# Xtra-Computing/FedTree

Hardware: AMD Instinct MI355X
Metric: Paillier-2048 encrypts/s device-resident; ciphertext adds/s; 1/2/4/8 GPU (higher is better)
Workload: dtype u32

## Files before the change

### fedtree_amd/build.py

```python
#!/usr/bin/env python3
import hashlib
import os
import subprocess
import sys

HERE = os.path.dirname(os.path.abspath(__file__))
CSRC = os.path.join(HERE, "csrc")
GEN = os.path.join(CSRC, "gen")
LLVM = "/opt/rocm/lib/llvm/bin"
ARCH = "gfx950"
VARIANTS = ((37, 28, 12, False), (74, 28, 12, False), (152, 27, 4, True), (80, 27, 4, True))
DEFAULT_OUT = os.path.join(HERE, "libfthe.so")
OUT = os.path.abspath(os.environ.get("FTHE_BUILD_OUT") or DEFAULT_OUT)


def run(cmd):
    r = subprocess.run(cmd, capture_output=True, text=True)
    if r.returncode != 0:
        sys.stderr.write(" ".join(cmd) + "\n" + r.stdout + r.stderr)
        raise SystemExit(r.returncode)
    return r


def build_kernels():
    os.makedirs(GEN, exist_ok=True)
    sys.path.insert(0, CSRC)
    if OUT == DEFAULT_OUT:
        for k in sorted(k for k in os.environ if k.startswith("FTHE_GEN_")):
            os.environ.pop(k)
            sys.stderr.write(f"build.py: ignoring {k} (A/B generator switch) for the in-tree library\n")
    import gen_montprog
    import gen_padic
    import gen_nadic
    import gen_padic_mfma
    import gen_addb
    import gen_nadicb
    for lay_name, new_lay in (("addb_layout.h", gen_addb.layout_header()), ("nadicb_layout.h", gen_nadicb.layout_header())):
        lay = os.path.join(GEN, lay_name)
        if not os.path.exists(lay) or open(lay).read() != new_lay:
            with open(lay, "w") as f:
                f.write(new_lay)
    blobs = []
    kernels = [(S, f"fthe_montprog_s{S}", f"montprog_s{S}",
                (lambda S=S, B=B, U=U, quad=quad, n=f"fthe_montprog_s{S}":
                 (gen_montprog.gen_quad if quad else gen_montprog.gen)(S, B, U, n)))
               for S, B, U, quad in VARIANTS]
    for K in (37, 19):
        kernels.append((1000 + K, f"fthe_padic_k{K}", f"padic_k{K}",
                        lambda K=K: gen_padic.gen_padic(K, 28, f"fthe_padic_k{K}")))
    kernels.append((1137, "fthe_padic_m37", "padic_m37", lambda: gen_padic_mfma.gen_padic_mfma("fthe_padic_m37")))
    kernels.append((1237, "fthe_padic_m37t", "padic_m37t",
                    lambda: gen_padic_mfma.gen_padic_mfma("fthe_padic_m37t", top_est=True)))
    kernels.append((2076, "fthe_nadic_q76", "nadic_q76", lambda: gen_nadic.gen_nadic(76, 27, "fthe_nadic_q76")))
    kernels.append((2176, "fthe_nadic_m76", "nadic_m76",
                    lambda: gen_nadic.gen_nadic(76, 27, "fthe_nadic_m76", mont=True)))
    kernels.append((2276, "fthe_nadic_b76", "nadic_b76", lambda: gen_nadicb.gen_nadicb("fthe_nadic_b76")))
    kernels.append((3152, "fthe_addb_q152", "addb_q152", lambda: gen_addb.gen_addb("fthe_addb_q152")))
    for S, name, stem, make in kernels:
        asm = os.path.join(GEN, f"{stem}.s")
        src = make()
        old = open(asm).read() if os.path.exists(asm) else None
        if old != src:
            with open(asm, "w") as f:
                f.write(src)
        obj = os.path.join(GEN, f"{stem}.o")
        hsaco = os.path.join(GEN, f"{stem}.hsaco")
        run([f"{LLVM}/clang", "-x", "assembler", "-target", "amdgcn-amd-amdhsa", f"-mcpu={ARCH}",
             "-c", asm, "-o", obj])
        run([f"{LLVM}/ld.lld", "-shared", obj, "-o", hsaco])
        blobs.append((S, open(hsaco, "rb").read()))
    hdr = ["// generated by fedtree_amd/build.py -- gfx950 code objects of the montprog kernels",
           "#pragma once", "#include <cstddef>", ""]
    for S, b in blobs:
        hdr.append(f"alignas(64) static const unsigned char fthe_blob_s{S}[{len(b)}] = {{")
        for i in range(0, len(b), 24):
            hdr.append("  " + ",".join(str(x) for x in b[i:i + 24]) + ",")
        hdr.append("};")
    hdr.append("static inline const unsigned char *fthe_montprog_blob(int S) {")
    for S, _ in blobs:
        hdr.append(f"  if (S == {S}) return fthe_blob_s{S};")
    hdr.append("  return nullptr;")
    hdr.append("}")
    path = os.path.join(GEN, "montprog_blobs.h")
    new = "\n".join(hdr) + "\n"
    if not os.path.exists(path) or open(path).read() != new:
        with open(path, "w") as f:
            f.write(new)


def build_lib():
    srcs = [os.path.join(CSRC, "fthe.hip"), os.path.join(CSRC, "fthe_glue.hip"), os.path.join(CSRC, "fthe_hist.hip"),
            os.path.join(CSRC, "fthe_dec.hip"), os.path.join(CSRC, "fthe_wire.cpp")]
    deps = srcs + [os.path.join(CSRC, f) for f in ("bn_host.hpp", "fthe_glue.h", "padic_tiles.hpp", "addb_image.hpp",
                                                    "nadicb_image.hpp")] + \
        [os.path.join(GEN, "montprog_blobs.h"), os.path.join(GEN, "addb_layout.h"), os.path.join(GEN, "nadicb_layout.h"),
         os.path.join(HERE, "..", "include", "fthe.h")]
    cmd = ["/opt/rocm/bin/hipcc", f"--offload-arch={ARCH}", "-O3", "-fPIC", "-shared", "-std=c++17",
           "-idirafter", "/opt/conda/include", "-Wno-unused-result",
           *(["-DFTHE_STAMP_HOOK"] if OUT != DEFAULT_OUT else []),
           *srcs, "-l:libgmp.so.10", "-o", OUT + ".tmp"]
    h = hashlib.sha256(" ".join(cmd[:-2]).encode())
    for d in deps:
        with open(d, "rb") as f:
            h.update(os.path.basename(d).encode() + b"\0" + f.read())
    digest = h.hexdigest()
# ... 18 lines not shown
```

### fedtree_amd/csrc/fthe.hip

```cpp
#include <hip/hip_runtime.h>
#include <cstdio>
#include <cstdlib>
#include <cstring>
#include <algorithm>
#include <atomic>
#include <cmath>
#include <chrono>
#include <condition_variable>
#include <functional>
#include <map>
#include <memory>
#include <string>
#include <mutex>
#include <new>
#include <random>
#include <thread>
#include <unordered_map>
#include <vector>
#include <fcntl.h>
#include <unistd.h>

#include "../../include/fthe.h"
#include "bn_host.hpp"
#include "padic_tiles.hpp"
#include "addb_image.hpp"
#include "nadicb_image.hpp"
#include "fthe_glue.h"
#include "gen/montprog_blobs.h"

using namespace fthe;

#define HIPOK(x) do { if ((x) != hipSuccess) return FTHE_ERR_HIP; } while (0)

namespace {

constexpr int MAX_VARIANTS = 11;
constexpr int kPadicS = 1037, kPadicK = 37, kPadicSmallK = 19, kNadicS = 2076, kPadicMfmaS = 1137,
              kNadicMontS = 2176, kNadicBarS = 2276, kPadicMfmaTS = 1237;
constexpr int kPadicTopBits = 1027, kPadicPtShift = 1000, kPadicPtWord = 100;
const Shape kVariants[MAX_VARIANTS] = {{37, 28, 1}, {74, 28, 1}, {152, 27, 4}, {80, 27, 4},
                                       {1000 + kPadicK, 28, 1}, {1000 + kPadicSmallK, 28, 1}, {kNadicS, 27, 4},
                                       {kPadicMfmaS, 28, 1}, {kNadicMontS, 27, 4}, {kNadicBarS, 27, 4},
                                       {kPadicMfmaTS, 28, 1}};
constexpr Shape kLatShape{80, 27, 4};
constexpr int kAddbBlob = 3152;

int variant_index(int S) {
    for (int i = 0; i < MAX_VARIANTS; i++) if (kVariants[i].S == S) return i;
    return -1;
}

void urandom_bytes(void *dst, size_t n) {
    uint8_t *p = (uint8_t *)dst;
    size_t got = 0;
    int fd = open("/dev/urandom", O_RDONLY);
    if (fd >= 0) {
        while (got < n) {
            ssize_t r = read(fd, p + got, n - got);
            if (r <= 0) break;
            got += (size_t)r;
        }
        close(fd);
    }
    if (got < n) {
        std::random_device rd;
        for (; got < n; got++) p[got] = (uint8_t)rd();
    }
}

uint64_t splitmix64(uint64_t &s) {
    uint64_t z = (s += 0x9E3779B97F4A7C15ull);
    z = (z ^ (z >> 30)) * 0xBF58476D1CE4E5B9ull;
    z = (z ^ (z >> 27)) * 0x94D049BB133111EBull;
    return z ^ (z >> 31);
}

RngKey make_rng_key(uint64_t seed, uint64_t tweak) {
    RngKey rk{};
    if (!seed) {
        urandom_bytes(rk.k, sizeof rk.k);
        urandom_bytes(&rk.nonce, sizeof rk.nonce);
        return rk;
    }
    uint64_t s = seed;
    for (int i = 0; i < 8; i += 2) { uint64_t v = splitmix64(s); rk.k[i] = (uint32_t)v; rk.k[i + 1] = (uint32_t)(v >> 32); }
    rk.nonce = splitmix64(s) ^ tweak;
    return rk;
}

void seed_gmp_state(gmp_randstate_t st, uint64_t seed, uint64_t tweak) {
    Mpz sd;
    if (!seed) {
        uint32_t w[8];
        urandom_bytes(w, sizeof w);
        mpz_import(sd, 8, -1, 4, 0, 0, w);
    } else {
// ... 330 lines not shown
static bool lds_prefetch(const Shape &sh) {
    static const bool off = getenv("FTHE_NO_LDSDMA") != nullptr;
    return sh.lanes == 1 && !off;
}

extern "C" int fthe_version(void) { return 100; }

extern "C" const char *fthe_strerror(int s) {
    switch (s) {
        case FTHE_OK: return "ok";
        case FTHE_ERR_ARG: return "invalid argument";
        case FTHE_ERR_HIP: return "HIP runtime error (no gfx950 device or launch failure)";
        case FTHE_ERR_NOPRIV: return "private key required";
        case FTHE_ERR_UNSUPPORTED: return "modulus size not supported by the built kernels";
        case FTHE_ERR_KEY: return "invalid key material";
        case FTHE_ERR_NOMEM: return "device allocation failed";
        default: return "unknown status";
    }
}

extern "C" int fthe_kernel_limbs(int bits) { return kernel_limbs_for_bits(bits); }

extern "C" int fthe_device_count(void) {
    int n = 0;
    return hipGetDeviceCount(&n) == hipSuccess && n > 0 ? n : 0;
}

extern "C" int fthe_ctx_create(int device, fthe_ctx **out) {
    if (!out) return FTHE_ERR_ARG;
    *out = nullptr;
    int ndev = 0;
    if (hipGetDeviceCount(&ndev) != hipSuccess || ndev <= 0 || device < 0 || device >= ndev) return FTHE_ERR_HIP;
    HIPOK(hipSetDevice(device));
    std::unique_ptr<fthe_ctx> c(new fthe_ctx);
    c->device = device;
    HIPOK(hipStreamCreateWithFlags(&c->stream, hipStreamNonBlocking));
    HIPOK(hipStreamCreateWithFlags(&c->copy, hipStreamNonBlocking));
    HIPOK(hipStreamCreateWithFlags(&c->side, hipStreamNonBlocking));
    HIPOK(hipEventCreateWithFlags(&c->ev_fork, hipEventDisableTiming));
    HIPOK(hipEventCreateWithFlags(&c->ev_join, hipEventDisableTiming));
    for (int i = 0; i < 2; i++) {
        HIPOK(hipEventCreateWithFlags(&c->ev_done[i], hipEventDisableTiming));
        HIPOK(hipEventCreateWithFlags(&c->ev_copied[i], hipEventDisableTiming));
        HIPOK(hipEventCreateWithFlags(&c->ev_in[i], hipEventDisableTiming));
    }
    for (int i = 0; i < MAX_VARIANTS; i++) {
        const unsigned char *blob = fthe_montprog_blob(kVariants[i].S);
        if (!blob) return FTHE_ERR_HIP;
        HIPOK(hipModuleLoadData(&c->mod[i], blob));
        char name[64];
        if (kVariants[i].S > 2200) snprintf(name, sizeof name, "fthe_nadic_b%d", kVariants[i].S - 2200);
        else if (kVariants[i].S > 2100) snprintf(name, sizeof name, "fthe_nadic_m%d", kVariants[i].S - 2100);
        else if (kVariants[i].S > 2000) snprintf(name, sizeof name, "fthe_nadic_q%d", kVariants[i].S - 2000);
        else if (kVariants[i].S > 1200) snprintf(name, sizeof name, "fthe_padic_m%dt", kVariants[i].S - 1200);
        else if (kVariants[i].S > 1100) snprintf(name, sizeof name, "fthe_padic_m%d", kVariants[i].S - 1100);
        else if (kVariants[i].S > 1000) snprintf(name, sizeof name, "fthe_padic_k%d", kVariants[i].S - 1000);
        else snprintf(name, sizeof name, "fthe_montprog_s%d", kVariants[i].S);
        HIPOK(hipModuleGetFunction(&c->fn[i], c->mod[i], name));
        HIPOK(hipFuncGetAttribute(&c->static_lds[i], HIP_FUNC_ATTRIBUTE_SHARED_SIZE_BYTES, c->fn[i]));
    }
    if (const unsigned char *blob = fthe_montprog_blob(kAddbBlob)) {
        HIPOK(hipModuleLoadData(&c->mod_addb, blob));
        HIPOK(hipModuleGetFunction(&c->fn_addb, c->mod_addb, "fthe_addb_q152"));
    }
    HIPOK(hipEventCreate(&c->ev0));
    HIPOK(hipEventCreate(&c->ev1));
    HIPOK(hipDeviceGetAttribute(&c->n_cu, hipDeviceAttributeMultiprocessorCount, device));
    *out = c.release();
    return FTHE_OK;
}

extern "C" int fthe_host_alloc(size_t bytes, void **out) {
    if (!out) return FTHE_ERR_ARG;
    *out = nullptr;
    if (bytes == 0) return FTHE_OK;
    if (hipHostMalloc(out, bytes, hipHostMallocDefault) != hipSuccess) { *out = nullptr; return FTHE_ERR_HIP; }
    return FTHE_OK;
}

extern "C" void fthe_host_free(void *p) {
    if (p) (void)hipHostFree(p);
}

extern "C" void fthe_ctx_destroy(fthe_ctx *c) {
    if (!c) return;
    (void)hipSetDevice(c->device);
    if (c->stream) (void)hipStreamSynchronize(c->stream);
    if (c->copy) (void)hipStreamSynchronize(c->copy);
    if (c->side) (void)hipStreamSynchronize(c->side);
    for (int i = 0; i < MAX_VARIANTS; i++) if (c->mod[i]) (void)hipModuleUnload(c->mod[i]);
    if (c->mod_addb) (void)hipModuleUnload(c->mod_addb);
    if (c->d_jobctr) (void)hipFree(c->d_jobctr);
    if (c->cub_tmp) (void)hipFree(c->cub_tmp);
    for (auto &e : c->prof_ev) { (void)hipEventDestroy(e.first); (void)hipEventDestroy(e.second); }
    if (c->ev0) (void)hipEventDestroy(c->ev0);
    if (c->ev1) (void)hipEventDestroy(c->ev1);
    if (c->stream) (void)hipStreamDestroy(c->stream);
    if (c->copy) (void)hipStreamDestroy(c->copy);
    if (c->side) (void)hipStreamDestroy(c->side);
    if (c->ev_fork) (void)hipEventDestroy(c->ev_fork);
    if (c->ev_join) (void)hipEventDestroy(c->ev_join);
    for (int i = 0; i < 2; i++) {
        if (c->ev_done[i]) (void)hipEventDestroy(c->ev_done[i]);
        if (c->ev_copied[i]) (void)hipEventDestroy(c->ev_copied[i]);
        if (c->ev_in[i]) (void)hipEventDestroy(c->ev_in[i]);
    }
// ... 24 lines not shown
}
extern "C" double fthe_last_montmuls(fthe_ctx *c) { return c ? c->last_mm : 0.0; }

extern "C" int fthe_prof_variant(fthe_ctx *c, int S, double *expo_ms, double *expo_launches) {
    if (!c) return FTHE_ERR_ARG;
    int vi = variant_index(S);
    if (vi < 0) return FTHE_ERR_ARG;
    if (expo_ms) *expo_ms = c->var_ms[vi];
    if (expo_launches) *expo_launches = c->var_n[vi];
    return FTHE_OK;
}

extern "C" int fthe_prof_enable(fthe_ctx *c, int on) {
    if (!c) return FTHE_ERR_ARG;
    c->prof = on != 0;
    c->prof_used = 0; c->prof_lane_mm = 0; c->prof_launch_lanes = 0; c->prof_alg_macs = 0;
    c->prof_exec_macs = 0;
    return FTHE_OK;
}

extern "C" int fthe_prof_busy(fthe_ctx *c, double *busy_ms, double *expo_busy_ms) {
    if (!c) return FTHE_ERR_ARG;
    if (busy_ms) *busy_ms = c->prof_busy_ms;
    if (expo_busy_ms) *expo_busy_ms = c->prof_expo_busy_ms;
    return FTHE_OK;
}

extern "C" int fthe_prof_exec_macs(fthe_ctx *c, double *exec_macs) {
    if (!c || !exec_macs) return FTHE_ERR_ARG;
    HIPOK(hipSetDevice(c->device));
    HIPOK(hipStreamSynchronize(c->stream));
    *exec_macs = c->prof_exec_macs;
    return FTHE_OK;
}

extern "C" int fthe_prof_read(fthe_ctx *c, double *kernel_ms, double *launches, double *lane_montmuls, double *lanes,
                              double *expo_ms, double *expo_launches, double *alg_macs) {
    if (!c) return FTHE_ERR_ARG;
    HIPOK(hipSetDevice(c->device));
    HIPOK(hipStreamSynchronize(c->stream));
    HIPOK(hipStreamSynchronize(c->side));
    double tot = 0, etot = 0, en = 0;
    for (int v = 0; v < MAX_VARIANTS; v++) c->var_ms[v] = c->var_n[v] = 0;
    std::vector<std::pair<double, double>> iv, eiv;
    for (size_t i = 0; i < c->prof_used; i++) {
        float ms = 0, t0 = 0;
        HIPOK(hipEventElapsedTime(&ms, c->prof_ev[i].first, c->prof_ev[i].second));
        HIPOK(hipEventElapsedTime(&t0, c->prof_ev[0].first, c->prof_ev[i].first));
        tot += ms;
        iv.emplace_back(t0, (double)t0 + ms);
        if (c->prof_mm[i] >= 64) {
            etot += ms; en += 1;
            c->var_ms[c->prof_vi[i]] += ms; c->var_n[c->prof_vi[i]] += 1;
            if (kVariants[c->prof_vi[i]].S == kPadicMfmaTS) {
                const int vm = variant_index(kPadicMfmaS);
                c->var_ms[vm] += ms; c->var_n[vm] += 1;
            }
            eiv.emplace_back(t0, (double)t0 + ms);
        }
    }
    auto union_ms = [](std::vector<std::pair<double, double>> &v) {
        std::sort(v.begin(), v.end());
        double u = 0, a = 0, b = -1e300;
        for (auto &x : v) {
            if (x.first > b) { if (b > a) u += b - a; a = x.first; b = x.second; }
            else b = std::max(b, x.second);
        }
        if (!v.empty() && b > a) u += b - a;
        return u;
    };
    c->prof_busy_ms = union_ms(iv);
    c->prof_expo_busy_ms = union_ms(eiv);
    if (kernel_ms) *kernel_ms = tot;
    if (expo_ms) *expo_ms = etot;
    if (expo_launches) *expo_launches = en;
    if (launches) *launches = (double)c->prof_used;
    if (lane_montmuls) *lane_montmuls = c->prof_lane_mm;
    if (lanes) *lanes = c->prof_launch_lanes;
    if (alg_macs) *alg_macs = c->prof_alg_macs;
    c->prof_used = 0; c->prof_lane_mm = 0; c->prof_launch_lanes = 0; c->prof_alg_macs = 0; c->prof_exec_macs = 0;
    return FTHE_OK;
}

static int upload_mod(DevMod &d, const mpz_t N, Shape sh) {
    d.m.init(N, sh);
    if (hipMalloc(&d.d_ctx, d.m.ctx.size() * 4) != hipSuccess) return FTHE_ERR_NOMEM;
    HIPOK(hipMemcpy(d.d_ctx, d.m.ctx.data(), d.m.ctx.size() * 4, hipMemcpyHostToDevice));
    return FTHE_OK;
}

static int padic_digits(const mpz_t P, Shape sh) {
    if (getenv("FTHE_NO_PADIC") || sh.B != 28 || sh.lanes != 1) return 0;
    const size_t b = mpz_sizeinbase(P, 2);
    if (sh.S == 2 * kPadicK && b >= 1009 && b <= 1030) return kPadicK;
    if (sh.S == 37 && b >= 505 && b <= 516) return kPadicSmallK;
    return 0;
}
static int upload_padic(DevMod &d, const mpz_t P, int K) {
    Mpz P2; mpz_mul(P2, P, P);
    d.m.init(P2, Shape{2 * K, 28, 1});
    const int pad = ((20 + K + 3) & ~3) - 20 - K;
    std::vector<uint8_t> tiles;
    if (K == kPadicK && !getenv("FTHE_NO_PADIC_MFMA")) tiles = padic_tiles::build(P);
    std::vector<uint32_t> w(tiles.empty() ? (size_t)2 * K + 1 + pad : 128 + tiles.size() / 4, 0u), l = to_limbs(P, K, 28);
    if (!tiles.empty()) std::memcpy(w.data() + 128, tiles.data(), tiles.size());
    for (int j = 0; j < K; j++) w[j] = (uint32_t)(-(int32_t)l[j]);
    Mpz mu; mpz_set_ui(mu, 1); mpz_mul_2exp(mu, mu, 56 * K); mpz_fdiv_q(mu, mu, P);
    std::vector<uint32_t> ml = to_limbs(mu, K + 1, 28);
    std::copy(ml.begin(), ml.end(), w.begin() + K + pad);
    if (!tiles.empty()) {
        static_assert(kPadicPtWord >= 2 * kPadicK + 1 + 3 && kPadicPtWord < 128, "Pt between mu and the tile image");
        Mpz pt; mpz_fdiv_q_2exp(pt, P, kPadicPtShift);
        w[kPadicPtWord] = (uint32_t)mpz_get_ui(pt);
    }
    if (hipMalloc(&d.d_ctx, w.size() * 4) != hipSuccess) return FTHE_ERR_NOMEM;
    HIPOK(hipMemcpy(d.d_ctx, w.data(), w.size() * 4, hipMemcpyHostToDevice));
    d.kernel_S = 1000 + K;
    const bool top_est = !tiles.empty() && mpz_sizeinbase(P, 2) <= (size_t)kPadicTopBits && !getenv("FTHE_NO_M37T");
    d.kernel_S_mfma = tiles.empty() ? 0 : top_est ? kPadicMfmaTS : kPadicMfmaS;
    return FTHE_OK;
}
static double padic_alg(const Prog &p, const mpz_t P) {
    const double s = (double)((mpz_sizeinbase(P, 2) + 31) / 32);
    const double bar = (s + 1) * (s + 2) / 2 + s * (s + 1) / 2;
    const double sq = s * s + s * (s + 1) / 2 + 2 * bar, mul = 3 * s * s + 2 * bar;
    return p.squarings * sq + (p.montmuls - p.squarings) * mul + bar + s * s;
}
static double padic_exec(const Prog &p, int Kd) {
    const double K = Kd;
    const double bar = K * (K + 1) + 3 * K + 1;
    const double sq = K * K + K * (K + 1) / 2 + 2 * bar, mul = 3 * K * K + 2 * bar;
    return p.squarings * sq + (p.montmuls - p.squarings) * mul + bar + K * K + K;
}

constexpr Shape kNadicDigit{76, 27, 4};
static bool nadic_ok(const fthe_key *k) {
    const size_t b = mpz_sizeinbase(k->n, 2);
    return !getenv("FTHE_NO_NADIC") && k->sn2.S == 152 && k->sn2.B == 27 && k->sn2.lanes == 4 &&
           b >= 2042 && b <= 2050;
}
static bool nadic_mont_ok(const fthe_key *k) {
    return !getenv("FTHE_NO_NADIC") && !getenv("FTHE_NADIC_CLASSICAL") && k->sn2.S == 152 && k->sn2.B == 27 &&
           k->sn2.lanes == 4 && mpz_sizeinbase(k->n, 2) <= 2048;
}
static bool nadicb_ok(const fthe_key *k) {
    return !getenv("FTHE_NO_NADIC") && !getenv("FTHE_NADIC_MONT") && !getenv("FTHE_NADIC_CLASSICAL") &&
           k->sn2.S == 152 && k->sn2.B == 27 && k->sn2.lanes == 4 && nadicb::n_ok(k->n);
}
static int upload_nadic(DevMod &d, const mpz_t n, const mpz_t n2, Shape slots, bool classical = true) {
    d.m.init(n2, slots);
    MontMod dm;
    dm.init(n, kNadicDigit);
    if (classical && !dm.classical_ok()) return FTHE_ERR_UNSUPPORTED;
    if (hipMalloc(&d.d_ctx, dm.ctx.size() * 4) != hipSuccess) return FTHE_ERR_NOMEM;
    HIPOK(hipMemcpy(d.d_ctx, dm.ctx.data(), dm.ctx.size() * 4, hipMemcpyHostToDevice));
    d.kernel_S = kNadicS;
    return FTHE_OK;
}
static double nadic_alg(const Prog &p, const mpz_t n) {
    const double s = (double)((mpz_sizeinbase(n, 2) + 31) / 32);
    return p.squarings * 4 * s * s + (p.montmuls - p.squarings) * 5 * s * s;
}
static double nadic_exec(const Prog &p) {
    return p.squarings * 76.0 * 76 + (p.montmuls - p.squarings) * 76.0 * 95;
}

static int key_finish(fthe_key *k) {
    if (k->priv) {
        Mpz p2; mpz_mul(p2, k->p, k->p);
        Mpz q2; mpz_mul(q2, k->q, k->q);
        size_t b = std::max(p2.bits(), q2.bits());
        k->spq = kernel_shape_for_bits((int)b);
// ... 3294 lines not shown
```

### fedtree_amd/csrc/gen_padic_mfma.py

```python
#!/usr/bin/env python3
import os
import sys

sys.path.insert(0, os.path.dirname(os.path.abspath(__file__)))
from gen_montprog import _descriptor

AB = os.environ.get("FTHE_GEN_M37_AB", "")
TILE_OFF = 512
TILE_BYTES = 20 * 1024
SPILL_BYTES = 10 * 1024
SPILL = "spill" in AB
PP = "pingpong" in AB
MARGIN = next((int(t[6:]) for t in AB.split(',') if t.startswith('margin') and t[6:].isdigit()), 30)
assert MARGIN >= 24
PREXOR = "noprexor" not in AB
CMERGE = "nocmerge" not in AB
LDSX = "ldsx" in AB
LDSXA = LDSX and "ldsxa" in AB
LDSX_BYTES = 5 * 1024
KARA = "nokara" not in AB
assert not (KARA and LDSX)
assert not (LDSX and (PP or SPILL))
LDS_BYTES = TILE_BYTES + (4 * SPILL_BYTES if SPILL else 0) + (4 * LDSX_BYTES if LDSX else 0)
S1_LO = 112 if "s1lo112" in AB else 128
S1_TOP = 272
Q3DW = "noq3dw" not in AB and not LDSX
QBIT = 28 * 38
TILE_D1 = (-3, -2, -1, 0, 1)
TILE_D2 = (0, 1, 2, 3)


def tile_index(prod, m, k):
    if prod == 1:
        return TILE_D1.index(m - k) if k <= 3 else 5 + m
    return 10 + m if k == 0 else 15 + TILE_D2.index(m - k)


TOPEST_MAX_BITS = 1027
PT_OFF = 400
PT_SHIFT = 1000
TOPEST_C = 128 << 8


def gen_padic_mfma(name: str, top_est: bool = False) -> str:
    K, B = 37, 28
    MASK = (1 << B) - 1
    V_TID, V_GOFF = 0, 1
    VA = (2, 6, 10)
    NCOL = next((int(t[3:]) for t in AB.split(',') if t in ('col3', 'col4')), 2)
    assert NCOL == 2 or not KARA, "col3 / col4 predate the Karatsuba cross term (wrong results, r06s): add nokara"
    ACC0 = 10 if NCOL == 2 else 2
    CARRY = ACC0 + 4 * NCOL
    XA = 20
    G0, G1 = XA, XA + 16
    XB = 60
    TT = 100
    VV = 174
    V_LDS = 248
    V_SPILL = 249
    PATV = (249, 250)
    assert not (SPILL and PREXOR)
    NVGPR = 250 if SPILL else 251 if PREXOR else 249
    V_XW, V_XR = NVGPR, NVGPR + 1
    if LDSX:
        NVGPR += 2

    def pat(t):
        return f"v{PATV[t % 2]}"
    PATVAL = (0x00808080, 0x08080808)
    X0 = [f"v{XA + i}" for i in range(K)]
    X1 = [f"v{XB + i}" for i in range(K)]
    T = [f"v{TT + i}" for i in range(2 * K)]
    V = [f"v{VV + i}" for i in range(2 * K)]
    D = [f"v{XB + i}" for i in range(40)]
    SPOW, SNEG, SNP = 20, 28, 36
    NSGPR = SNP + K
    SLO, SHI = 74, 76
    if LDSX:
        NSGPR = SHI + 2
    if KARA:
        NSGPR = 79
    SPT = NSGPR
    if top_est:
        NSGPR += 1
    POW = lambda sh: f"s{SPOW + sh // 4}"
    NEG = lambda sh: f"s{SNEG + sh // 4}"
    NP = lambda j: f"s{SNP + j}"

    def pair(n):
        return f"v[{n}:{n + 1}]"

    def acc(s, ch):
        n = ACC0 + 2 * (NCOL * s + ch)
        return f"v[{n}:{n + 1}]"

    def acclo(s, ch):
        return f"v{ACC0 + 2 * (NCOL * s + ch)}"

    carry = pair(CARRY)
# ... 77 lines not shown
            used = [False] * len(seqs)
            for ci in range(gi + NCOL, min(gi + 2 * NCOL, len(cols))):
                pending += list(cols[ci].get('pre', ()))
            n = 0
            for t in range(max(len(q[1]) for q in seqs)):
                for k, (ac, terms, add) in enumerate(seqs):
                    if t < len(terms):
                        a_, b_ = terms[t]
                        e(f'  {mad} {ac}, vcc, {a_}, {b_}, {ac if used[k] else (add or "0")}')
                        used[k] = True
                        n += 1
                        if n % 2 == 0:
                            tick()
            flush(len(pending))
            tail = []
            for m, ci in enumerate(members):
                tail += tail_of(ci, cols[ci], acc(s, m), acclo(s, m), used[m])
            pending = tail
        flush(len(pending))
        for ins in bgq:
            e(ins)

    def product_cols(a, b, n_out, outs, a2=None, b2=None):
        cols = []
        for c in range(n_out):
            terms = []
            for i in range(len(a)):
                j = c - i
                if 0 <= j < len(b):
                    terms.append((a[i], b[j]))
                    if a2 is not None:
                        terms.append((a2[i], b2[j]))
            cols.append({'terms': terms, 'out': outs[c], 'last': c == n_out - 1})
            if PREXOR and c >= K:
                cols[-1]['px'] = pat(c - (K - 1))
        return cols

    def move(dst, src):
        n = len(src)
        for i in range(0, n - 1, 2):
            if int(dst[i][1:]) % 2 == 0 and int(src[i][1:]) % 2 == 0:
                e(f'  v_pk_mov_b32 {pair(int(dst[i][1:]))}, {pair(int(src[i][1:]))}, {pair(int(src[i][1:]))} op_sel:[0,1]')
            else:
                e(f'  v_mov_b32_e32 {dst[i]}, {src[i]}')
                e(f'  v_mov_b32_e32 {dst[i + 1]}, {src[i + 1]}')
        if n % 2:
            e(f'  v_mov_b32_e32 {dst[n - 1]}, {src[n - 1]}')

    CACC2 = (pair(XA + 32), pair(XA + 34))
    CCARRY = pair(XA + 38)
    SMASK = "s35"
    S2MASK, S3MASK, S4MASK = "s76", "s77", "s78"

    def orpack(limbs, shift_bits, ndw, xor_masks, lead_one=False, norm0=False, pre=()):
        n = len(limbs)
        pre = set(pre)

        def carried(w):
            m = 0
            for b in range(32):
                q = 32 * w - shift_bits + b
                if q < 0 or (lead_one and w == 0 and b < 8):
                    continue
                t, j = q // B, q % B
                if t in pre and t < n and (PATVAL[t % 2] >> j) & 1:
                    m |= 1 << b
            return m
        xor_masks = [xor_masks[w] ^ carried(w) for w in range(ndw)]
        for w in range(ndw):
            d = D[w]
            if lead_one and w == 0:
                e(f'  v_lshl_or_b32 {d}, {limbs[0]}, 8, 1')
            else:
                lo = (32 * w - shift_bits) // B
                off = 32 * w - shift_bits - B * lo
                hi_ok = lo + 1 < n
                if norm0 and lo == 0:
                    assert off == 0 and hi_ok
                    e(f'  v_lshlrev_b32_e32 {d}, 28, {limbs[1]}')
                    e(f'  v_bfi_b32 {d}, {SMASK}, {limbs[0]}, {d}')
                elif not hi_ok:
                    e(f'  v_lshrrev_b32_e32 {d}, {off}, {limbs[lo]}')
                elif off == 0:
                    e(f'  v_lshl_or_b32 {d}, {limbs[lo + 1]}, 28, {limbs[lo]}')
                else:
                    e(f'  v_lshrrev_b32_e32 {d}, {off}, {limbs[lo]}')
                    e(f'  v_lshl_or_b32 {d}, {limbs[lo + 1]}, {B - off}, {d}')
            if xor_masks[w]:
                e(f'  v_xor_b32_e32 {d}, {hex(xor_masks[w])}, {d}')

    D2 = [f"v{VV + 38 + i}" for i in range(36)] + [f"v{16 + i}" for i in range(4)]
    OPND = [D]

    def swap_operands(Dl=D, nk=5):
        if LDSX:
            assert nk == 5
            lo, hi = f"s[{SLO}:{SLO + 1}]", f"s[{SHI}:{SHI + 1}]"
            e(f'  s_mov_b64 exec, {lo}')
            for k in range(5):
                e(f'  ds_write_b128 v{V_XW}, v[{XB + 8 * k + 4}:{XB + 8 * k + 7}] offset:{1024 * k}')
            e(f'  s_mov_b64 exec, {hi}')
            for k in range(5):
                e(f'  ds_write_b128 v{V_XW}, v[{XB + 8 * k}:{XB + 8 * k + 3}] offset:{1024 * k}')
            for k in range(5):
                e(f'  ds_read_b128 v[{XB + 8 * k}:{XB + 8 * k + 3}], v{V_XR} offset:{1024 * k}')
            e(f'  s_mov_b64 exec, {lo}')
            for k in range(5):
                e(f'  ds_read_b128 v[{XB + 8 * k + 4}:{XB + 8 * k + 7}], v{V_XR} offset:{1024 * k}')
            e('  s_mov_b64 exec, -1')
            return
        e('  s_nop 1')
        for k in range(nk):
            for j in range(4):
                e(f'  v_permlane32_swap_b32_e32 {Dl[8 * k + j]}, {Dl[8 * k + 4 + j]}')
        e('  s_nop 4')

    def rd(prod, m, k, n):
        b_ = VA[n % 3]
        e(f'  ds_read_b128 v[{b_}:{b_ + 3}], v{V_LDS} offset:{1024 * tile_index(prod, m, k)}')

    def prefetch(prod, m, ks):
        for n in range(min(2, len(ks))):
            rd(prod, m, ks[n], n)

    GB0, GB1 = TT + 38, TT + 54
    GV0, GV1 = VV + 38, VV + 54

    def issue_tile(prod, m, ks, G0x, G1x, prefetched=True):
        L = len(ks)
        if not prefetched:
            prefetch(prod, m, ks)
        for n, k in enumerate(ks):
            if n + 2 < L:
                rd(prod, m, ks[n + 2], n + 2)
            e(f'  s_waitcnt lgkmcnt({min(L, n + 3) - n - 1})')
            buf = VA[n % 3]
            for g, G in ((0, G0x), (1, G1x)):
                src_c = "0" if n == 0 else f"v[{G}:{G + 15}]"
                bo = 8 * k + 4 * g
                b0 = int(OPND[0][bo][1:])
                assert b0 % 2 == 0 and [int(r[1:]) for r in OPND[0][bo:bo + 4]] == list(range(b0, b0 + 4))
                if "nomfma" not in AB:
                    e(f'  v_mfma_i32_32x32x32_i8 v[{G}:{G + 15}], v[{buf}:{buf + 3}], v[{b0}:{b0 + 3}], {src_c}')

    P1_TOP = [S1_TOP]

    def consumed(prod, m):
        if prod == 1:
            return {rho for rho in range(32) if S1_LO + 32 * m + rho < P1_TOP[0]}
        return {rho for rho in range(32) if 1 <= 32 * m + rho <= 130}

    def plan(C):
        paired, swaps = set(), []
        for rr in range(0, 16, 2):
            ra = 8 * (rr >> 2) + (rr & 3)
            rhos = (ra, ra + 4)
            if "noprepair" not in AB and all((r in C) == (r + 1 in C) for r in rhos) \
                    and any(r in C for r in rhos):
                paired.add(rr)
        for rr in range(16):
            ra = 8 * (rr >> 2) + (rr & 3)
            if (ra in C or ra + 4 in C) and not (rr % 2 and rr - 1 in paired):
                swaps.append(rr)
        return paired, swaps

    def compact(tile):
        return LDSXA and plan(consumed(*tile))[0] == set(range(0, 16, 2))

    def exchange(G0x, G1x, waited=False, tile=None):
        if "nonop" not in AB and not waited:
            e('  s_nop 7')
            e('  s_nop 7')
# ... 143 lines not shown
                tail += self.out(self.t, f'v{a[2:a.index(":")]}')
            elif 0 <= self.t < len(self.outs):
                if self.px:
                    tail.append(f'  v_bitop3_b32 {self.outs[self.t]}, v{a[2:a.index(":")]}, {SMASK}, '
                                f'{pat(self.t)} bitop3:0x6a')
                else:
                    tail.append(f'  v_and_b32_e32 {self.outs[self.t]}, {hex(MASK)}, v{a[2:a.index(":")]}')
            if not (self.nocarry_last and self.t == self.t_last):
                if CMERGE:
                    e(f'  v_ashrrev_i64 {CCARRY}, {self.radix}, {a}')
                else:
                    tail.append(f'  v_ashrrev_i64 {CCARRY}, {self.radix}, {a}')
            self.pending = tail
            self.t += 1
            self.fresh = True
            if self.t <= self.t_last:
                self.start()

        def column(self, s, reg):
            t = (8 * s - self.base) // self.radix
            while t > self.t:
                self.close()
            if not self.begun:
                self.begun = True
                self.start()
            sh = 8 * s - self.base - self.radix * t
            mul = NEG(sh) if self.neg else POW(sh)
            a = self.acc()
            self.emit(f'  v_mad_i64_i32 {a}, vcc, {reg}, {mul}, {self.addend0() if self.fresh else a}')
            self.fresh = False

        def finish(self):
            while self.t <= self.t_last:
                self.close()
            for ins in self.pending:
                e(ins)
            self.pending = []

    def fold_columns(ch, cols):
        i = 0
        while i < len(cols):
            s_, r_, pr_ = cols[i]
            if not pr_ and i + 1 < len(cols) and "nopair" not in AB:
                s2_, r2_, pr2_ = cols[i + 1]
                t1, t2 = (8 * s_ - ch.base) // ch.radix, (8 * s2_ - ch.base) // ch.radix
                if not pr2_ and s2_ == s_ + 1 and t1 == t2 and 8 * s_ - ch.base - ch.radix * t1 <= 16:
                    e(f'  v_lshl_add_u32 {r_}, {r2_}, 8, {r_}')
                    ch.column(s_, r_)
                    i += 2
                    continue
            ch.column(s_, r_)
            i += 1

    P1_TILES = [(1, m, [k for k in range(5) if m - k <= 1]) for m in range(5)]
    P2_TILES = [(2, m, [k for k in range(5) if m >= k]) for m in range(5)]
    assert P1_TILES[0][2][0] != 4 and P2_TILES[0][2][0] != 4

    V_FRAC = XA + 37
    assert V_FRAC not in range(G0, G0 + 32) and V_FRAC not in range(XA + 32, XA + 37) and \
        V_FRAC not in (XA + 38, XA + 39) and V_FRAC < XB and V_FRAC >= CARRY + 2 and V_FRAC not in VA

    def mfma_barrett(Tl, q3out, clamp, prefetched=False, dbuf=False, setb=None, pre_in=None, dw=None, t4=False):
        if pre_in is None:
            pre_in = PREXOR
        if not prefetched:
            prefetch(*P1_TILES[0])
        orpack(Tl[K - 1:2 * K], 0, 34, [0x80808080] * 34, norm0=True, pre=range(1, K + 1) if pre_in else ())
        e(f'  v_bfe_u32 {D[34]}, {Tl[K - 1]}, 28, 1')
        e(f'  v_lshl_or_b32 {D[34]}, {D[34]}, 12, 1')
        for w in range(35, 40):
            e(f'  v_mov_b32_e32 {D[w]}, 0')
        swap_operands()
        if dw is None:
            tap = {-1: lambda lo: [f'  v_lshlrev_b32_e32 v{V_FRAC}, 4, {lo}']} if t4 else None
            ch = Chunks(QBIT, (8 * S1_LO - QBIT) // B, 39, q3out, neg=False, px=PREXOR, tap=tap)
        else:
            assert not clamp
            base = QBIT - 8

            ndw = 32 if t4 else 33
            tap = {-1: lambda lo: [f'  v_mov_b32_e32 v{V_FRAC}, {lo}'],
                   0: lambda lo: [f'  v_alignbit_b32 v{V_FRAC}, {lo}, v{V_FRAC}, 8']} if t4 else None

            def out(w, lo):
                if w < 0:
                    return []
                if w == 0:
                    return [f'  v_and_b32_e32 {dw[0]}, 0xffffff00, {lo}', f'  v_xor_b32_e32 {dw[0]}, 0x80808001, {dw[0]}']
                if w == 32:
                    return [f'  v_and_b32_e32 {dw[32]}, {hex((1 << (B * K + 8 - 1024)) - 1)}, {lo}',
                            f'  v_xor_b32_e32 {dw[32]}, 0x80808080, {dw[32]}']
                return [f'  v_xor_b32_e32 {dw[w]}, 0x80808080, {lo}']
            ch = Chunks(base, (8 * S1_LO - base) // 32, ndw - 1, None, neg=False, nocarry_last=True, radix=32,
                        out=out, tap=tap)
            P1_TOP[0] = (base + ndw * 32) // 8

        def consume(m, creg):
            fold_columns(ch, tile_cols(1, m, lambda rho: S1_LO + 32 * m + rho, creg))
        run_tiles(P1_TILES, consume, P2_TILES[0], dbuf, setb=setb)
        ch.finish()
        P1_TOP[0] = S1_TOP
        if clamp:
            e(f'  v_not_b32_e32 v{XA + 36}, v{XA + 38}')
            for t, r in enumerate(q3out):
                if PREXOR:
                    e(f'  v_bitop3_b32 {r}, {r}, v{XA + 36}, {pat(t)} bitop3:0xe2')
                else:
                    e(f'  v_and_b32_e32 {r}, {r}, v{XA + 36}')
        return q3out

    def mfma_remainder(Tl, q3, rout, nxt_p1, dbuf=False, after_pack=None, dw=None, t4=False, clamped=False):
        Dl = D if dw is None else dw
        nk = 4 if t4 else 5
        if dw is None:
            orpack(q3, 8, 32 if t4 else 33, [0x80808000] + [0x80808080] * 32, lead_one=True,
                   pre=range(K) if PREXOR else ())
        if after_pack and not dbuf:
            after_pack()
        if not t4:
            e(f'  v_mov_b32_e32 {Dl[33]}, 0x80')
            for w in range(34, 40):
                e(f'  v_mov_b32_e32 {Dl[w]}, 0')
        swap_operands(Dl, nk)
        OPND[0] = Dl
# ... 343 lines not shown
        e('  s_waitcnt vmcnt(0)')
        e('.Lstamp_done:')
    e('  s_endpgm')

    e('.Lreduce:')
    PRIO = next((int(t[4:]) for t in AB.split(',') if t.startswith('prio') and t[4:].isdigit()),
                0 if "noprio" in AB else 3)
    if PRIO:
        e(f'  s_setprio {PRIO}')
    dbuf = "nodbuf" not in AB
    spill = dbuf and SPILL
    if spill:
        for j in range(9):
            e(f'  ds_write_b128 v{V_SPILL}, v[{VV + 38 + 4 * j}:{VV + 41 + 4 * j}] offset:{1024 * j}')
        e(f'  ds_write_b32 v{V_SPILL}, {V[K]} offset:{9 * 1024}')
    q3 = mfma_barrett(T, T[K:], clamp=True, dbuf=spill, setb=(GV0, GV1), t4=top_est)

    def add_u1():
        for i in range(K):
            if PREXOR:
                e(f'  v_xad_u32 {V[i]}, {q3[i]}, {pat(i)}, {V[i]}')
            else:
                e(f'  v_add_u32_e32 {V[i]}, {V[i]}, {q3[i]}')
        if spill:
            for j in range(9):
                e(f'  ds_read_b128 v[{VV + 38 + 4 * j}:{VV + 41 + 4 * j}], v{V_SPILL} offset:{1024 * j}')
            e(f'  ds_read_b32 {V[K]}, v{V_SPILL} offset:{9 * 1024}')
    mfma_remainder(T, q3, T[:K], nxt_p1=True, dbuf=dbuf, after_pack=add_u1, t4=top_est, clamped=True)
    if Q3DW:
        mfma_barrett(V, None, clamp=False, prefetched=True, dbuf=dbuf, dw=D2, t4=top_est)
        mfma_remainder(V, None, V[:K], nxt_p1=False, dbuf=dbuf, dw=D2, t4=top_est)
    else:
        q3b = mfma_barrett(V, V[K:], clamp=False, prefetched=True, dbuf=dbuf, t4=top_est)
        mfma_remainder(V, q3b, V[:K], nxt_p1=False, dbuf=dbuf, t4=top_est)
    move(X0, T[:K])
    move(X1, V[:K])
    if PRIO:
        e('  s_setprio 0')
    e('  s_setpc_b64 s[12:13]')

    e(f'.Lfunc_end_{name}:')
    e(f'  .size {name}, .Lfunc_end_{name}-{name}')
    e('')
    o.extend(_descriptor(name, LDS_BYTES, NVGPR, 98 if DYN else 90 if STAMP else NSGPR,
                         max_wg=512 if PP else 256).splitlines())
    return "\n".join(o) + "\n"


if __name__ == "__main__":
    import argparse
    ap = argparse.ArgumentParser()
    ap.add_argument('--name', default='fthe_padic_m37')
    ap.add_argument('--top-est', action='store_true', help='the four-tile body (fthe_padic_m37t)')
    ap.add_argument('-o', '--out', required=True)
    a = ap.parse_args()
    with open(a.out, 'w') as f:
        f.write(gen_padic_mfma(a.name, top_est=a.top_est))
```

### fedtree_amd/csrc/padic_tiles.hpp

```cpp
#pragma once
#include <gmp.h>
#include <cstdint>
#include <vector>

namespace padic_tiles {

constexpr int kTiles = 19, kImageBytes = 20 * 1024, kS1Lo = 128, kNq1 = 136, kConst1 = 136, kNq3 = 132;

inline bool balanced(const mpz_t x, int n, std::vector<int> &d) {
    mpz_t t;
    mpz_init_set(t, x);
    d.assign(n, 0);
    int c = 0;
    for (int k = 0; k < n; k++) {
        int v = (int)(mpz_get_ui(t) & 255u) + c;
        mpz_fdiv_q_2exp(t, t, 8);
        if (v >= 128) { d[k] = v - 256; c = 1; } else { d[k] = v; c = 0; }
    }
    bool ok = mpz_sgn(t) == 0 && c == 0;
    mpz_clear(t);
    return ok;
}

inline void offset_sum(mpz_t out, const mpz_t x, int n) {
    mpz_t g;
    mpz_init(g);
    mpz_ui_pow_ui(g, 256, (unsigned long)n);
    mpz_sub_ui(g, g, 1);
    mpz_divexact_ui(g, g, 255);
    mpz_mul(out, g, x);
    mpz_mul_ui(out, out, 128);
    mpz_clear(g);
}

inline std::vector<uint8_t> build(const mpz_t P, int s1lo = kS1Lo) {
    std::vector<uint8_t> img;
    if (mpz_sizeinbase(P, 2) < 1009 || mpz_sizeinbase(P, 2) > 1030) return img;
    if (s1lo != 112 && s1lo != 128) return img;
    mpz_t mu, c, b;
    mpz_inits(mu, c, b, nullptr);
    mpz_set_ui(mu, 1);
    mpz_mul_2exp(mu, mu, 56 * 37);
    mpz_fdiv_q(mu, mu, P);
    std::vector<int> mud, pd, g1, g2;
    bool ok = balanced(mu, 135, mud) && balanced(P, 130, pd);
    offset_sum(c, mu, kNq1);
    mpz_set_ui(b, 1);
    mpz_mul_2exp(b, b, 8 * s1lo + 22);
    mpz_sub(c, c, b);
    mpz_fdiv_q_2exp(c, c, 8 * s1lo);
    ok = ok && balanced(c, 160, g1);
    offset_sum(c, P, kNq3);
    mpz_fdiv_r_2exp(c, c, 1040);
    ok = ok && balanced(c, 131, g2);
    mpz_clears(mu, c, b, nullptr);
    if (!ok) return img;
    g2.resize(130);
    auto a1 = [&](int s, int i) -> int {
        if (i == kConst1) return (s >= s1lo && s < s1lo + 160) ? g1[s - s1lo] : 0;
        if (i == kConst1 + 1) {
            int j = s - 3;
            return (j >= 0 && j < (int)mud.size()) ? mud[j] : 0;
        }
        if (i > kConst1) return 0;
        int j = s - i;
        return (j >= 0 && j < (int)mud.size()) ? mud[j] : 0;
    };
    auto a2 = [&](int s, int i) -> int {
        if (i == 0) return (s >= 1 && s <= (int)g2.size()) ? g2[s - 1] : 0;
        int j = s - i;
        return (j >= 0 && j < (int)pd.size()) ? pd[j] : 0;
    };
    img.reserve(kImageBytes);
    auto tile = [&](int prod, int s_base, int m, int k) {
        for (int l = 0; l < 64; l++) {
            const int r = l & 31, h = l >> 5;
            for (int j = 0; j < 16; j++) {
                const int s = s_base + 32 * m + r, i = 32 * k + 16 * h + j;
                img.push_back((uint8_t)((prod == 1 ? a1(s, i) : a2(s, i)) & 255));
            }
        }
    };
    for (int d = -3; d <= 1; d++) tile(1, s1lo, d >= 0 ? d : 0, d >= 0 ? 0 : -d);
    for (int m = 0; m < 5; m++) tile(1, s1lo, m, 4);
    for (int m = 0; m < 5; m++) tile(2, 0, m, 0);
    for (int d = 0; d <= 3; d++) tile(2, 0, d + 1, 1);
    img.resize(kImageBytes, 0);
    return img;
}

}
```

Before: 2.927 million.

## Add shifted-operand p-adic MFMA kernel that drops the first-product superdiagonal tiles

```diff
diff --git a/fedtree_amd/build.py b/fedtree_amd/build.py
--- a/fedtree_amd/build.py
+++ b/fedtree_amd/build.py
@@ -51,6 +51,9 @@
     kernels.append((1137, "fthe_padic_m37", "padic_m37", lambda: gen_padic_mfma.gen_padic_mfma("fthe_padic_m37")))
     kernels.append((1237, "fthe_padic_m37t", "padic_m37t",
                     lambda: gen_padic_mfma.gen_padic_mfma("fthe_padic_m37t", top_est=True)))
+    kernels.append((1337, "fthe_padic_m37s", "padic_m37s",
+                    lambda: gen_padic_mfma.gen_padic_mfma("fthe_padic_m37s", top_est=True,
+                                                          q1_shift=gen_padic_mfma.Q1_SHIFT)))
     kernels.append((2076, "fthe_nadic_q76", "nadic_q76", lambda: gen_nadic.gen_nadic(76, 27, "fthe_nadic_q76")))
     kernels.append((2176, "fthe_nadic_m76", "nadic_m76",
                     lambda: gen_nadic.gen_nadic(76, 27, "fthe_nadic_m76", mont=True)))
diff --git a/fedtree_amd/csrc/fthe.hip b/fedtree_amd/csrc/fthe.hip
--- a/fedtree_amd/csrc/fthe.hip
+++ b/fedtree_amd/csrc/fthe.hip
@@ -34,14 +34,14 @@
 
 namespace {
 
-constexpr int MAX_VARIANTS = 11;
+constexpr int MAX_VARIANTS = 12;
 constexpr int kPadicS = 1037, kPadicK = 37, kPadicSmallK = 19, kNadicS = 2076, kPadicMfmaS = 1137,
-              kNadicMontS = 2176, kNadicBarS = 2276, kPadicMfmaTS = 1237;
+              kNadicMontS = 2176, kNadicBarS = 2276, kPadicMfmaTS = 1237, kPadicMfmaSS = 1337;
 constexpr int kPadicTopBits = 1027, kPadicPtShift = 1000, kPadicPtWord = 100;
 const Shape kVariants[MAX_VARIANTS] = {{37, 28, 1}, {74, 28, 1}, {152, 27, 4}, {80, 27, 4},
                                        {1000 + kPadicK, 28, 1}, {1000 + kPadicSmallK, 28, 1}, {kNadicS, 27, 4},
                                        {kPadicMfmaS, 28, 1}, {kNadicMontS, 27, 4}, {kNadicBarS, 27, 4},
-                                       {kPadicMfmaTS, 28, 1}};
+                                       {kPadicMfmaTS, 28, 1}, {kPadicMfmaSS, 28, 1}};
 constexpr Shape kLatShape{80, 27, 4};
 constexpr int kAddbBlob = 3152;
 
@@ -478,6 +478,7 @@
         if (kVariants[i].S > 2200) snprintf(name, sizeof name, "fthe_nadic_b%d", kVariants[i].S - 2200);
         else if (kVariants[i].S > 2100) snprintf(name, sizeof name, "fthe_nadic_m%d", kVariants[i].S - 2100);
         else if (kVariants[i].S > 2000) snprintf(name, sizeof name, "fthe_nadic_q%d", kVariants[i].S - 2000);
+        else if (kVariants[i].S > 1300) snprintf(name, sizeof name, "fthe_padic_m%ds", kVariants[i].S - 1300);
         else if (kVariants[i].S > 1200) snprintf(name, sizeof name, "fthe_padic_m%dt", kVariants[i].S - 1200);
         else if (kVariants[i].S > 1100) snprintf(name, sizeof name, "fthe_padic_m%d", kVariants[i].S - 1100);
         else if (kVariants[i].S > 1000) snprintf(name, sizeof name, "fthe_padic_k%d", kVariants[i].S - 1000);
@@ -608,9 +609,14 @@
         if (c->prof_mm[i] >= 64) {
             etot += ms; en += 1;
             c->var_ms[c->prof_vi[i]] += ms; c->var_n[c->prof_vi[i]] += 1;
-            if (kVariants[c->prof_vi[i]].S == kPadicMfmaTS) {
+            const int vs = kVariants[c->prof_vi[i]].S;
+            if (vs == kPadicMfmaTS || vs == kPadicMfmaSS) {
                 const int vm = variant_index(kPadicMfmaS);
                 c->var_ms[vm] += ms; c->var_n[vm] += 1;
+            }
+            if (vs == kPadicMfmaSS) {
+                const int vt = variant_index(kPadicMfmaTS);
+                c->var_ms[vt] += ms; c->var_n[vt] += 1;
             }
             eiv.emplace_back(t0, (double)t0 + ms);
         }
@@ -657,7 +663,10 @@
     d.m.init(P2, Shape{2 * K, 28, 1});
     const int pad = ((20 + K + 3) & ~3) - 20 - K;
     std::vector<uint8_t> tiles;
-    if (K == kPadicK && !getenv("FTHE_NO_PADIC_MFMA")) tiles = padic_tiles::build(P);
+    const bool top_ok = mpz_sizeinbase(P, 2) <= (size_t)kPadicTopBits && !getenv("FTHE_NO_M37T");
+    const bool shifted = top_ok && !getenv("FTHE_NO_M37S");
+    if (K == kPadicK && !getenv("FTHE_NO_PADIC_MFMA"))
+        tiles = padic_tiles::build(P, padic_tiles::kS1Lo, shifted ? padic_tiles::kQShift : 0);
     std::vector<uint32_t> w(tiles.empty() ? (size_t)2 * K + 1 + pad : 128 + tiles.size() / 4, 0u), l = to_limbs(P, K, 28);
     if (!tiles.empty()) std::memcpy(w.data() + 128, tiles.data(), tiles.size());
     for (int j = 0; j < K; j++) w[j] = (uint32_t)(-(int32_t)l[j]);
@@ -672,8 +681,7 @@
     if (hipMalloc(&d.d_ctx, w.size() * 4) != hipSuccess) return FTHE_ERR_NOMEM;
     HIPOK(hipMemcpy(d.d_ctx, w.data(), w.size() * 4, hipMemcpyHostToDevice));
     d.kernel_S = 1000 + K;
-    const bool top_est = !tiles.empty() && mpz_sizeinbase(P, 2) <= (size_t)kPadicTopBits && !getenv("FTHE_NO_M37T");
-    d.kernel_S_mfma = tiles.empty() ? 0 : top_est ? kPadicMfmaTS : kPadicMfmaS;
+    d.kernel_S_mfma = tiles.empty() ? 0 : shifted ? kPadicMfmaSS : top_ok ? kPadicMfmaTS : kPadicMfmaS;
     return FTHE_OK;
 }
 static double padic_alg(const Prog &p, const mpz_t P) {
diff --git a/fedtree_amd/csrc/gen_padic_mfma.py b/fedtree_amd/csrc/gen_padic_mfma.py
--- a/fedtree_amd/csrc/gen_padic_mfma.py
+++ b/fedtree_amd/csrc/gen_padic_mfma.py
@@ -30,8 +30,11 @@
 TILE_D2 = (0, 1, 2, 3)
 
 
-def tile_index(prod, m, k):
+def tile_index(prod, m, k, q1_shift=0):
     if prod == 1:
+        if q1_shift and k == 0:
+            assert m == 0
+            return 4
         return TILE_D1.index(m - k) if k <= 3 else 5 + m
     return 10 + m if k == 0 else 15 + TILE_D2.index(m - k)
 
@@ -42,9 +45,14 @@
 TOPEST_C = 128 << 8
 
 
-def gen_padic_mfma(name: str, top_est: bool = False) -> str:
+Q1_SHIFT = 8
+
+
+def gen_padic_mfma(name: str, top_est: bool = False, q1_shift: int = 0) -> str:
     K, B = 37, 28
     MASK = (1 << B) - 1
+    assert q1_shift in (0, Q1_SHIFT) and not (q1_shift and (LDSX or S1_LO != 128))
+    QD = q1_shift // 4
     V_TID, V_GOFF = 0, 1
     VA = (2, 6, 10)
     NCOL = next((int(t[3:]) for t in AB.split(',') if t in ('col3', 'col4')), 2)
@@ -228,7 +236,7 @@
     SMASK = "s35"
     S2MASK, S3MASK, S4MASK = "s76", "s77", "s78"
 
-    def orpack(limbs, shift_bits, ndw, xor_masks, lead_one=False, norm0=False, pre=()):
+    def orpack(limbs, shift_bits, ndw, xor_masks, lead_one=False, norm0=False, pre=(), d0=0):
         n = len(limbs)
         pre = set(pre)
 
@@ -244,7 +252,7 @@
             return m
         xor_masks = [xor_masks[w] ^ carried(w) for w in range(ndw)]
         for w in range(ndw):
-            d = D[w]
+            d = D[w + d0]
             if lead_one and w == 0:
                 e(f'  v_lshl_or_b32 {d}, {limbs[0]}, 8, 1')
             else:
@@ -293,7 +301,7 @@
 
     def rd(prod, m, k, n):
         b_ = VA[n % 3]
-        e(f'  ds_read_b128 v[{b_}:{b_ + 3}], v{V_LDS} offset:{1024 * tile_index(prod, m, k)}')
+        e(f'  ds_read_b128 v[{b_}:{b_ + 3}], v{V_LDS} offset:{1024 * tile_index(prod, m, k, q1_shift)}')
 
     def prefetch(prod, m, ks):
         for n in range(min(2, len(ks))):
@@ -543,7 +551,7 @@
             ch.column(s_, r_)
             i += 1
 
-    P1_TILES = [(1, m, [k for k in range(5) if m - k <= 1]) for m in range(5)]
+    P1_TILES = [(1, m, [k for k in range(5) if m - k <= (0 if q1_shift else 1)]) for m in range(5)]
     P2_TILES = [(2, m, [k for k in range(5) if m >= k]) for m in range(5)]
     assert P1_TILES[0][2][0] != 4 and P2_TILES[0][2][0] != 4
 
@@ -556,11 +564,13 @@
             pre_in = PREXOR
         if not prefetched:
             prefetch(*P1_TILES[0])
-        orpack(Tl[K - 1:2 * K], 0, 34, [0x80808080] * 34, norm0=True, pre=range(1, K + 1) if pre_in else ())
-        e(f'  v_bfe_u32 {D[34]}, {Tl[K - 1]}, 28, 1')
-        e(f'  v_lshl_or_b32 {D[34]}, {D[34]}, 12, 1')
-        for w in range(35, 40):
-            e(f'  v_mov_b32_e32 {D[w]}, 0')
+        orpack(Tl[K - 1:2 * K], 0, 34, [0x80808080] * 34, norm0=True, pre=range(1, K + 1) if pre_in else (), d0=QD)
+        DC = D[34 + QD]
+        e(f'  v_bfe_u32 {DC}, {Tl[K - 1]}, 28, 1')
+        e(f'  v_lshl_or_b32 {DC}, {DC}, 12, 1')
+        if not q1_shift:
+            for w in range(35, 40):
+                e(f'  v_mov_b32_e32 {D[w]}, 0')
         swap_operands()
         if dw is None:
             tap = {-1: lambda lo: [f'  v_lshlrev_b32_e32 v{V_FRAC}, 4, {lo}']} if t4 else None
@@ -1010,7 +1020,8 @@
     ap = argparse.ArgumentParser()
     ap.add_argument('--name', default='fthe_padic_m37')
     ap.add_argument('--top-est', action='store_true', help='the four-tile body (fthe_padic_m37t)')
+    ap.add_argument('--q1-shift', type=int, default=0, help='8 with --top-est: the shifted operand (fthe_padic_m37s)')
     ap.add_argument('-o', '--out', required=True)
     a = ap.parse_args()
     with open(a.out, 'w') as f:
-        f.write(gen_padic_mfma(a.name, top_est=a.top_est))
+        f.write(gen_padic_mfma(a.name, top_est=a.top_est, q1_shift=a.q1_shift))
diff --git a/fedtree_amd/csrc/padic_tiles.hpp b/fedtree_amd/csrc/padic_tiles.hpp
--- a/fedtree_amd/csrc/padic_tiles.hpp
+++ b/fedtree_amd/csrc/padic_tiles.hpp
@@ -5,7 +5,7 @@
 
 namespace padic_tiles {
 
-constexpr int kTiles = 19, kImageBytes = 20 * 1024, kS1Lo = 128, kNq1 = 136, kConst1 = 136, kNq3 = 132;
+constexpr int kTiles = 19, kImageBytes = 20 * 1024, kS1Lo = 128, kNq1 = 136, kConst1 = 136, kNq3 = 132, kQShift = 8;
 
 inline bool balanced(const mpz_t x, int n, std::vector<int> &d) {
     mpz_t t;
@@ -33,10 +33,11 @@
     mpz_clear(g);
 }
 
-inline std::vector<uint8_t> build(const mpz_t P, int s1lo = kS1Lo) {
+inline std::vector<uint8_t> build(const mpz_t P, int s1lo = kS1Lo, int qshift = 0) {
     std::vector<uint8_t> img;
     if (mpz_sizeinbase(P, 2) < 1009 || mpz_sizeinbase(P, 2) > 1030) return img;
     if (s1lo != 112 && s1lo != 128) return img;
+    if (qshift != 0 && (qshift != kQShift || s1lo != 128)) return img;
     mpz_t mu, c, b;
     mpz_inits(mu, c, b, nullptr);
     mpz_set_ui(mu, 1);
@@ -57,6 +58,8 @@
     if (!ok) return img;
     g2.resize(130);
     auto a1 = [&](int s, int i) -> int {
+        i -= qshift;
+        if (i < 0) return 0;
         if (i == kConst1) return (s >= s1lo && s < s1lo + 160) ? g1[s - s1lo] : 0;
         if (i == kConst1 + 1) {
             int j = s - 3;
@@ -81,7 +84,12 @@
             }
         }
     };
-    for (int d = -3; d <= 1; d++) tile(1, s1lo, d >= 0 ? d : 0, d >= 0 ? 0 : -d);
+    if (qshift) {
+        for (int d = -3; d <= 0; d++) tile(1, s1lo, d + 3, 3);
+        tile(1, s1lo, 0, 0);
+    } else {
+        for (int d = -3; d <= 1; d++) tile(1, s1lo, d >= 0 ? d : 0, d >= 0 ? 0 : -d);
+    }
     for (int m = 0; m < 5; m++) tile(1, s1lo, m, 4);
     for (int m = 0; m < 5; m++) tile(2, 0, m, 0);
     for (int d = 0; d <= 3; d++) tile(2, 0, d + 1, 1);
```

Measured after the change: 2.980 million, median of 6. +1.8%, better.
